# SeanNobel/DALLE2-video

Hardware: AMD Instinct MI355X
Metric: Unet3D denoise-steps/sec, 16f×64×64 clip bs=4; 1/2/4/8 MI355X (higher is better)
Workload: dtype bf16; 1 GPU; BASELINE config 2: unet1 (dim 64, mults 1/2/4/8) train step on a 16x64x64 clip, bs=4 per GPU: p_losses fwd+bwd + RCCL grad all-reduce + fused AdamW; batch_per_gpu=4, global_batch=4, parallelism=dp1

## Files before the change

### dalle2-video_amd/csrc/dv_conv.hip

```cpp
#include "dv_common.h"

#include <type_traits>

#include <algorithm>
#include <cstdlib>

using namespace dv;

#ifdef DV_STAMP
constexpr int DV_NSTAMP = 8;
__device__ unsigned long long g_dv_stamp[16384 * DV_NSTAMP];
#define DV_STAMP_AT(i)                                                                  \
  do {                                                                                  \
    if (threadIdx.x == 0) {                                                             \
      const long long blin = blockIdx.x + (long long)gridDim.x * (blockIdx.y + (long long)gridDim.y * blockIdx.z); \
      if (blin < 16384) g_dv_stamp[blin * DV_NSTAMP + (i)] = __builtin_amdgcn_s_memrealtime(); \
    }                                                                                   \
  } while (0)
extern "C" int dv_debug_stamps(unsigned long long* host, long long n) {
  if (n > 16384 * DV_NSTAMP) n = 16384 * DV_NSTAMP;
  return hipMemcpyFromSymbol(host, HIP_SYMBOL(g_dv_stamp), n * 8, 0, hipMemcpyDeviceToHost) == hipSuccess ? 0 : -1;
}
#else
#define DV_STAMP_AT(i) \
// ... 1908 lines not shown
    });
    if constexpr (GNIN) if (tr) {
      int ot = tid;
      asm volatile("" : "+v"(ot));
      const int gx = ot >> 3, gc = ot & 7;
#pragma unroll
      for (int i = 0; i < SEG; ++i) {
        const int q = (st + 1) * SEG + 2 + i, y = yq0 + q;
        const bool in = (unsigned)y < (unsigned)p.H;
        const u32x4 ov = in ? tv[i] : u32x4{0u, 0u, 0u, 0u};
        asm volatile("ds_write_b128 %0, %1" ::"v"(lds_addr(smem + (q % R) * ROWB + (gx + 1) * FS_XP + gc * 16)),
                     "v"(ov) : "memory");
        const bool own = in && q <= nst * SEG;
        __builtin_amdgcn_raw_buffer_store_b128(
            ov, yr, own ? (unsigned)(((fbase + y * W + gx) * p.gi_ldy + gc * 8) * 2) : DMA_OOB, 0, 0);
      }
    }
#ifdef DV_STAMP
    if (st == 1) {
      asm volatile("s_nop 0" : "+v"(acc));
      DV_S1(4);
    }
#endif
    const bool silu = p.act == DV_ACT_SILU;
    float sv[stats ? 32 : 1];
    const unsigned gba = lds_addr(gi_bias + ch * 32 + 4 * h);
#pragma unroll
    for (int g = 0; g < 4; ++g) {
      const int n = ch * 32 + 8 * g + 4 * h;
      float v[4];
#pragma unroll
      for (int e = 0; e < 4; ++e) v[e] = acc[4 * g + e];
      if constexpr (GNIN) {
        u32x4 gb = ds_read_b128_off<0>(gba + 32 * g);
        lgkm_wait_tied<0>(gb);
        const f32x4 bb = __builtin_bit_cast(f32x4, gb);
#pragma unroll
        for (int e = 0; e < 4; ++e) v[e] += bb[e];
      }
      if (silu) {
#pragma unroll
        for (int e = 0; e < 4; ++e) v[e] = silu_f(v[e]);
      }
      if (NRES > 0) {
#pragma unroll
        for (int e = 0; e < 4; ++e) v[e] += (float)rv[g][e];
      }
      if (NRES > 1) {
#pragma unroll
        for (int e = 0; e < 4; ++e) v[e] += (float)rv2[g][e];
      }
      store4<bf16>(p.y + m * p.ldy + co0 + n, v);
      if constexpr (stats) {
#pragma unroll
        for (int e = 0; e < 4; ++e) {
          const float q = stored<bf16>(v[e]);
          sv[4 * g + e] = q;
          sv[16 + 4 * g + e] = q * q;
        }
      }
    }
    if constexpr (stats) {
      rs_step<32, 16>(sv, r);
#pragma unroll
      for (int i = 0; i < 16; ++i) sacc[i] += sv[i];
    }
    if (st == 1) DV_S1(5);
    if constexpr (GNIN) {
      if (st + 2 < nst) {
        constexpr int B0 = Y0 + SEG + 4, B1 = 2 * SEG + 8;
        static_assert(B0 + NPW <= 63 && B1 + NPW <= 63, "stripe vmcnt immediate out of range");
        const bool d3 = st + 3 < nst;
        if (st == 0) {
          if (d3) asm volatile("s_waitcnt vmcnt(%0)" ::"n"(B0 + NPW) : "memory");
          else asm volatile("s_waitcnt vmcnt(%0)" ::"n"(B0) : "memory");
        } else {
          if (d3) asm volatile("s_waitcnt vmcnt(%0)" ::"n"(B1 + NPW) : "memory");
          else asm volatile("s_waitcnt vmcnt(%0)" ::"n"(B1) : "memory");
        }
      }
      if (tr) asm volatile("s_waitcnt lgkmcnt(0)" ::: "memory");
    } else if (st + 1 < nst) {
      constexpr int NR = 4 * NRES;
      constexpr int A0 = NR + 4, A1 = 2 * NR + 8, A2 = 2 * NR + 12;
      static_assert(A1 + 2 * NPW <= 63 && A2 + 2 * NPW <= 63, "stripe vmcnt immediate out of range");
      const int nd = (st + 2 < nst) + (st + 3 < nst);
      if (st == 0) {
        if (nd == 2) asm volatile("s_waitcnt vmcnt(%0)" ::"n"(A0 + 2 * NPW) : "memory");
        else if (nd == 1) asm volatile("s_waitcnt vmcnt(%0)" ::"n"(A0 + NPW) : "memory");
        else asm volatile("s_waitcnt vmcnt(%0)" ::"n"(A0) : "memory");
      } else if (st == 1) {
        if (nd == 2) asm volatile("s_waitcnt vmcnt(%0)" ::"n"(A1 + 2 * NPW) : "memory");
        else if (nd == 1) asm volatile("s_waitcnt vmcnt(%0)" ::"n"(A1 + NPW) : "memory");
        else asm volatile("s_waitcnt vmcnt(%0)" ::"n"(A1) : "memory");
      } else {
        if (nd == 2) asm volatile("s_waitcnt vmcnt(%0)" ::"n"(A2 + 2 * NPW) : "memory");
        else if (nd == 1) asm volatile("s_waitcnt vmcnt(%0)" ::"n"(A2 + NPW) : "memory");
        else asm volatile("s_waitcnt vmcnt(%0)" ::"n"(A2) : "memory");
      }
    }
    if (st == 1) DV_S1(6);
    __builtin_amdgcn_s_barrier();
    if (st == 0) DV_STAMP_AT(2);
    if (st == 1) DV_S1(7);
  }
  DV_STAMP_AT(3);
  if constexpr (stats) {
    __shared__ float red[2 * 64];
    rs_tail();
    if (nst > 0) gn_block_add<bf16, 32>(p, sacc, (long long)(sbeg + nst - 1) * 128 / p.gn_P, chan, red, co0, 64);
  }
}

bool fwd_stripe_ok(long long M, int h, int w, int cin, bool split, int cout, int ks, int ld0) {
  return ks == 3 && cin == 64 && !split && cout % 64 == 0 && (w == 32 || w == 64 || w == 128) &&
         h % (128 / w) == 0 && M % 128 == 0 && ld0 % 8 == 0 && M * ld0 * 2 < (long long)DMA_OOB;
}

int launch_fwd_stripe(const ConvFwdArgs<bf16>& a, hipStream_t st) {
  const int nstages = (int)(a.M / 128);
  const int ct = a.cout / 64;
  int bx = 256 / ct;
  if (bx < 1) bx = 1;
  if (bx > nstages) bx = nstages;
  const int spf = a.H / (128 / a.W);
  int sps = (nstages + bx - 1) / bx;
  if (sps >= spf) sps = spf;
  else while (spf % sps) ++sps;
  bx = (nstages + sps - 1) / sps;
  dim3 grid(bx, ct);
  const int nres = a.res2 ? 2 : a.res ? 1 : 0;
  const bool stats = a.gn_sums != nullptr;
  if (a.gi_sums) {
    if (stats) conv_fwd_stripe_kernel<64, 0, true, true><<<grid, 512, 0, st>>>(a, nstages, sps);
    else conv_fwd_stripe_kernel<64, 0, false, true><<<grid, 512, 0, st>>>(a, nstages, sps);
    return check_launch("conv_fwd_stripe_gn_in");
  }
#define DV_FS(WW, RR) (stats ? conv_fwd_stripe_kernel<WW, RR, true><<<grid, 512, 0, st>>>(a, nstages, sps) \
                             : conv_fwd_stripe_kernel<WW, RR, false><<<grid, 512, 0, st>>>(a, nstages, sps))
#define DV_FSR(WW) (nres == 2 ? (void)conv_fwd_stripe_kernel<WW, 2, false><<<grid, 512, 0, st>>>(a, nstages, sps) \
                    : nres == 1 ? (void)conv_fwd_stripe_kernel<WW, 1, false><<<grid, 512, 0, st>>>(a, nstages, sps) \
                                : DV_FS(WW, 0))
  if (a.W == 64 && nres == 1 && stats) conv_fwd_stripe_kernel<64, 1, true><<<grid, 512, 0, st>>>(a, nstages, sps);
  else if (a.W == 64) DV_FSR(64);
  else if (a.W == 128) DV_FSR(128);
  else DV_FSR(32);
#undef DV_FSR
#undef DV_FS
  return check_launch("conv_fwd_stripe");
}


bool stripe_geom(int h, int w, int& seg, int& nseg);

constexpr int F2_WP = 592;
constexpr int F2_XP = 80;

template <int W, bool STATS = false>
__global__ __launch_bounds__(512) void conv_fwd_stripe2_kernel(ConvFwdArgs<bf16> p, int seg, int nseg) {
  constexpr int WP = W + 2;
  constexpr int NWIN = W == 8 ? 200 : (128 / W + 2) * WP;
  constexpr int WB = 64 * F2_WP, XB = NWIN * F2_XP;
  constexpr int BUF = WB + XB;
  constexpr int NLW = (64 * 36 + 511) / 512;
  constexpr int NLX = (NWIN * 4 + 511) / 512;
  __shared__ __attribute__((aligned(16))) char smem[2 * BUF];

  const int tid = threadIdx.x, lane = tid & 63;
  const int wave = __builtin_amdgcn_readfirstlane(tid >> 6);
  const int pt = wave & 3, ch = wave >> 2;
  const int co0 = blockIdx.y * 64;
  const long long m0 = (long long)blockIdx.x * 128;
  const int HW = p.H * W, segrows = (seg + 2) * WP;
  const int y0 = nseg > 1 ? 0 : (int)((m0 % HW) / W);

  int w_src[NLW], w_dst[NLW];
#pragma unroll
  for (int i = 0; i < NLW; ++i) {
    const int idx = tid + 512 * i;
    const int row = idx / 36, c = idx - row * 36;
    const bool ok = row < 64;
    w_src[i] = ok ? (co0 + row) * p.K + (c >> 2) * p.cin + (c & 3) * 8 : -1;
    w_dst[i] = row * F2_WP + c * 16;
  }
  int x_off[NLX], x_ry[NLX], x_dst[NLX], x_c[NLX];
#pragma unroll
  for (int i = 0; i < NLX; ++i) {
    const int idx = tid + 512 * i;
    const int px = idx >> 2, c = idx & 3;
    const int sg = px / segrows, rem = px - sg * segrows;
    const int ry = rem / WP, rx = rem - ry * WP;
    const bool ok = px < NWIN && sg < nseg && rx >= 1 && rx <= W;
    x_ry[i] = ok ? ry - 1 : -(1 << 20);
    x_off[i] = sg * seg * W + (ry - 1) * W + (rx - 1);
    x_dst[i] = px < NWIN ? px * F2_XP + c * 16 : -1;
    x_c[i] = c * 8;
  }
  u32x4 rw[NLW], rx_[NLX];
  auto load = [&](int hc) {
    const int ci = hc * 32;
    const bool first = ci < p.c0;
    const bf16* xb = first ? p.x0 + ci : p.x1 + (ci - p.c0);
    const int ld = first ? p.ld0 : p.ld1;
#pragma unroll
    for (int i = 0; i < NLW; ++i)
      if (w_src[i] >= 0) rw[i] = *(const u32x4*)(p.w + w_src[i] + ci);
#pragma unroll
    for (int i = 0; i < NLX; ++i) {
      const bool in = (unsigned)(y0 + x_ry[i]) < (unsigned)p.H;
      rx_[i] = in ? *(const u32x4*)(xb + (m0 + x_off[i]) * ld + x_c[i]) : u32x4{0u, 0u, 0u, 0u};
    }
  };
  auto store = [&](int buf) {
    char* b = smem + buf * BUF;
#pragma unroll
    for (int i = 0; i < NLW; ++i)
      if (w_src[i] >= 0) *(u32x4*)(b + w_dst[i]) = rw[i];
#pragma unroll
    for (int i = 0; i < NLX; ++i)
      if (x_dst[i] >= 0) *(u32x4*)(b + WB + x_dst[i]) = rx_[i];
  };

  const int r = lane & 31, h = lane >> 5;
  const int px = pt * 32 + r;
  const int sl = px / (seg * W), rl = px - sl * seg * W;
  const int wrow = sl * segrows + (rl / W) * WP + rl % W;
  const int aofs = (ch * 32 + r) * F2_WP + h * 16;
  const int bofs = WB + wrow * F2_XP + h * 16;

  f32x16 acc[1][1];
#pragma unroll
  for (int e = 0; e < 16; ++e) acc[0][0][e] = 0.f;
  const int nhc = p.cin / 32;
  load(0);
  store(0);
  __syncthreads();
  for (int hc = 0; hc < nhc; ++hc) {
    if (hc + 1 < nhc) load(hc + 1);
    const char* b = smem + (hc & 1) * BUF;
#pragma unroll
    for (int d = 0; d < 9; ++d) {
      const int toff = ((d / 3) * WP + (d % 3)) * F2_XP;
#pragma unroll
      for (int ks = 0; ks < 2; ++ks) {
        const u32x4 av = *(const u32x4*)(b + aofs + (d * 32 + ks * 16) * 2);
        const u32x4 bv = *(const u32x4*)(b + bofs + toff + ks * 32);
        acc[0][0] = Mma<bf16>::run(av, bv, acc[0][0]);
      }
    }
    if (hc + 1 < nhc) store((hc + 1) & 1);
    __syncthreads();
  }
  conv_epilogue<bf16, 1, 1, STATS>(p, acc, m0 + pt * 32, co0 + ch * 32, r, h, m0, 128, co0, 64,
                                   (float*)smem);
}

bool fwd_stripe2_ok(long long M, int h, int w, int cin, int c0, bool split, int cout, int ks, int& seg,
                    int& nseg) {
  if (ks != 3 || cin % 32 || (split && c0 % 32) || cout % 64 || M % 128 || !stripe_geom(h, w, seg, nseg))
    return false;
  return w == 8 || (w == 16 && (long long)cin * cout <= 256 * 256);
}

int launch_fwd_stripe2(const ConvFwdArgs<bf16>& a, int seg, int nseg, hipStream_t st) {
  dim3 grid((unsigned)(a.M / 128), a.cout / 64);
  switch (a.W) {
#define DV_S2(WW) (a.gn_sums ? conv_fwd_stripe2_kernel<WW, true><<<grid, 512, 0, st>>>(a, seg, nseg) \
                          : conv_fwd_stripe2_kernel<WW, false><<<grid, 512, 0, st>>>(a, seg, nseg))
    case 64: DV_S2(64); break;
    case 32: DV_S2(32); break;
    case 16: DV_S2(16); break;
    default: DV_S2(8); break;
#undef DV_S2
  }
  return check_launch("conv_fwd_stripe2");
}

constexpr int F8_WROW = 19;
template <int W, int CO = 64, int NWV = 4, int NB = 0>
struct FwGeom {
  static constexpr int CG = CO * (NWV / 4);
  static constexpr int NF = W == 8 ? 2 : 1;
  static constexpr int NWR = W == 8 ? 10 : 128 / W + 2;
  static constexpr int WQ = W == 8 ? 12 : W + 2;
  static constexpr int FPIX = NWR * WQ;
  static constexpr int WPIX = NF * FPIX;
  static constexpr int XPIECES = (WPIX * 3 + 63) / 64;
  static constexpr int WPC = (CG * F8_WROW + 63) / 64;
  static constexpr int PIECES = WPC + XPIECES;
  static constexpr int NPW = (PIECES + NWV - 1) / NWV;
  static constexpr int BUF = PIECES * 1024;
  static constexpr int NBUF = NB ? NB : ((160 * 1024 - 1024) / BUF >= 5 ? 5 : (160 * 1024 - 1024) / BUF);
};

template <int W>
__device__ __forceinline__ int fw_pix(int r) {
  const bool ga = r < 4 || (r >= 12 && r < 16) || (r >= 20 && r < 28);
  const int a = ga ? (r < 4 ? r : (r < 16 ? r - 8 : r - 12))
                   : (r < 12 ? r - 4 : (r < 20 ? r - 8 : r - 16));
  if constexpr (W == 8) return (2 * (a >> 3) + (ga ? 0 : 1)) * 8 + (a & 7);
  else if constexpr (W == 16) return (ga ? 0 : 16) + a;
  else return (ga ? 0 : 16) + a;
}

template <int W, bool STATS = false, int PF = 2, int DEFER = 0, int CO = 64, bool SPLIT = true, int NWV = 4,
          bool TS = false>
__global__ __launch_bounds__(NWV * 64) void conv_fwd_frame_kernel(ConvFwdArgs<bf16> p) {
  using G = FwGeom<W, CO, TS ? 4 : NWV>;
  constexpr int PIECES = G::PIECES, BUF = G::BUF, NBUF = G::NBUF, WQ = G::WQ;
  constexpr int NPW = (PIECES + NWV - 1) / NWV;
  constexpr int WPC = G::WPC, NJ = TS ? 1 : CO / 32, CG = G::CG;
  static_assert(NWV == 4 || (NWV == 8 && (TS || !STATS)), "the 8-wave 2*CO tile has no statistics epilogue");
  static_assert(!TS || (NWV == 8 && CO == 64), "the tap split runs 8 waves on a 64-channel tile");
  static_assert(NPW <= 9, "one DMA piece per tap");
  __shared__ __attribute__((aligned(1024))) char smem[NBUF * BUF];
  DV_STAMP_AT(0);
  const int tid = threadIdx.x, lane = tid & 63;
  const int wave = __builtin_amdgcn_readfirstlane(tid >> 6) & (NWV - 1);
  const int wq = wave & 3;
  const int chh = TS ? 0 : wave >> 2;
  const int half = TS ? wave >> 2 : 0;
  const int npx = (int)(p.M / 128), nblk = npx * (p.cout / CG);
  int L = blockIdx.x;
  int co0;
  long long m0;
  if (p.xcd_c > 0) {
    const int xc = p.xcd_c, xp = 8 / xc, x = L % 8, j = L / 8;
    const int tpc = (p.cout / CG) / xc, ppg = npx / xp;
    co0 = ((x / xp) * tpc + j / ppg) * CG;
    m0 = (long long)((x % xp) * ppg + j % ppg) * 128;
  } else {
    if (nblk % 8 == 0) L = (L % 8) * (nblk / 8) + L / 8;
    co0 = (L / npx) * CG;
    m0 = (long long)(L % npx) * 128;
  }
  const int cbeg = 0, cend = p.cin / 16;
  const int nch = cend - cbeg;
  const int HW = p.H * W;
  const int y0 = W == 8 ? 0 : (int)((m0 % HW) / W);
  const long long fb = W == 8 ? m0 : m0 - (m0 % HW) + (long long)y0 * W;

  unsigned voff0[NPW], voff1[NPW];
#pragma unroll
  for (int i = 0; i < NPW; ++i) {
    const int k = min(wave + NWV * i, PIECES - 1);
    voff0[i] = voff1[i] = DMA_OOB;
    if (k < WPC) {
      const int slot = k * 64 + lane, row = slot / F8_WROW, c = slot - row * F8_WROW;
      if (c < 18 && row < CG) voff0[i] = (unsigned)((((long long)co0 + row) * p.K + c * 8) * 2);
    } else {
      const int slot = (k - WPC) * 64 + lane, px = slot / 3, s = slot - px * 3;
      const int f = px / G::FPIX, rem = px - f * G::FPIX, wy = rem / WQ, wx = rem - wy * WQ;
      const int y = y0 + wy - 1;
      if (px < G::WPIX && s < 2 && wx >= 1 && wx <= W && y >= 0 && y < p.H &&
          (W == 8 || wy <= 128 / W + 1)) {
        const long long pix = fb + (long long)f * 64 + (long long)(wy - 1) * W + (wx - 1);
        voff0[i] = (unsigned)(pix * p.ld0 * 2 + s * 16);
        voff1[i] = (unsigned)(pix * p.ld1 * 2 + s * 16);
      }
    }
  }
  const __amdgpu_buffer_rsrc_t wr = dma_rsrc(p.w, (unsigned)((long long)p.cout * p.K * 2));
  const __amdgpu_buffer_rsrc_t xr0 = dma_rsrc(p.x0, (unsigned)(p.M * p.ld0 * 2));
  const __amdgpu_buffer_rsrc_t xr1 = dma_rsrc(p.x1, (unsigned)(p.M * p.ld1 * 2));
  auto issue1 = [&](int c, int i) {
    const int ci0 = c * 16;
    const bool first = ci0 < p.c0;
    char* b = smem + (c % NBUF) * BUF;
    const int k = min(wave + NWV * i, PIECES - 1);
    if (k < WPC) dma16s(wr, b + k * 1024, voff0[i], (unsigned)ci0 * 18);
    else if (!SPLIT || first) dma16s(xr0, b + k * 1024, voff0[i], (unsigned)ci0 * 2);
    else dma16s(xr1, b + k * 1024, voff1[i], (unsigned)(ci0 - p.c0) * 2);
  };
  auto issue = [&](int c) {
#pragma unroll
    for (int i = 0; i < NPW; ++i) issue1(c, i);
  };
  constexpr int AHEAD = NBUF - 1;
#pragma unroll
  for (int c = 0; c < AHEAD; ++c)
    if (c < nch) issue(cbeg + c);
  {
    const int pro = min(AHEAD, nch) - 1;
    if (pro >= 3) asm volatile("s_waitcnt vmcnt(%0)" ::"n"(3 * NPW) : "memory");
    else if (pro == 2) asm volatile("s_waitcnt vmcnt(%0)" ::"n"(2 * NPW) : "memory");
    else if (pro == 1) asm volatile("s_waitcnt vmcnt(%0)" ::"n"(NPW) : "memory");
    else asm volatile("s_waitcnt vmcnt(0)" ::: "memory");
  }
  __builtin_amdgcn_s_barrier();
  DV_STAMP_AT(1);
#ifdef DV_STAMP
  unsigned long long st_wait = 0, st_bar = 0;
  const unsigned long long st_l0 = __builtin_amdgcn_s_memtime();
#endif

  const int r = lane & 31, h = lane >> 5;
  const int pix = fw_pix<W>(r);
  const int tpx = wq * 32 + pix;
  const int wb = W == 8 ? (tpx >> 6) * G::FPIX + ((tpx & 63) >> 3) * WQ + (tpx & 7)
                        : (tpx / W) * WQ + tpx % W;
  const int bofs = WPC * 1024 + (wb * 3 + h) * 16;
  const int aofs = (chh * CO + r) * (F8_WROW * 16) + h * 16;
  f32x16 acc0, acc1, acc2, acc3;
#pragma unroll
  for (int e = 0; e < 16; ++e) acc0[e] = acc1[e] = acc2[e] = acc3[e] = 0.f;
  static_assert(DEFER <= 2, "at most the last two taps are deferred");
  u32x4 lb[2], la0[2], la1[2];
  auto run_deferred = [&](auto HALF) {
    constexpr int D1 = TS && decltype(HALF)::value == 0 ? 5 : 9;
#pragma unroll
    for (int t = 0; t < DEFER; ++t) {
      const int tap = D1 - DEFER + t;
      if (tap & 1) {
        acc2 = Mma<bf16>::run(la0[t], lb[t], acc2);
        if (CO == 64) acc3 = Mma<bf16>::run(la1[t], lb[t], acc3);
      } else {
        acc0 = Mma<bf16>::run(la0[t], lb[t], acc0);
        if (CO == 64) acc1 = Mma<bf16>::run(la1[t], lb[t], acc1);
      }
    }
  };
  auto defer_wait = [&]() {
    if (DEFER == 2 && CO == 64)
      asm volatile("s_waitcnt lgkmcnt(0)" : "+v"(lb[0]), "+v"(la0[0]), "+v"(la1[0]), "+v"(lb[1]), "+v"(la0[1]),
                   "+v"(la1[1])::"memory");
    else if (DEFER == 2)
      asm volatile("s_waitcnt lgkmcnt(0)" : "+v"(lb[0]), "+v"(la0[0]), "+v"(lb[1]), "+v"(la0[1])::"memory");
    else if (DEFER && CO == 64)
      asm volatile("s_waitcnt lgkmcnt(0)" : "+v"(lb[0]), "+v"(la0[0]), "+v"(la1[0])::"memory");
    else if (DEFER)
      asm volatile("s_waitcnt lgkmcnt(0)" : "+v"(lb[0]), "+v"(la0[0])::"memory");
    else
      asm volatile("s_waitcnt lgkmcnt(0)" ::: "memory");
  };
  auto chunk = [&](int c, auto PRE, auto HALF) {
    const char* b = smem + (c % NBUF) * BUF;
    constexpr int D0 = TS && decltype(HALF)::value == 1 ? 5 : 0;
    constexpr int D1 = TS && decltype(HALF)::value == 0 ? 5 : 9;
    constexpr int NS = PF + 1;
    u32x4 bq[NS], aq0[NS], aq1[NS];
    auto rd = [&](int d, int s) {
      const int T = ((d / 3) * WQ + (d % 3)) * 48;
      bq[s] = *(const u32x4*)(b + bofs + T);
      aq0[s] = *(const u32x4*)(b + aofs + d * 32);
      if (CO == 64) aq1[s] = *(const u32x4*)(b + aofs + 32 * F8_WROW * 16 + d * 32);
    };
#pragma unroll
    for (int d = D0; d < D0 + PF; ++d) rd(d, d % NS);
    if (DEFER && c > cbeg) run_deferred(HALF);
#pragma unroll
    for (int d = D0; d < D1; ++d) {
      if (d + PF < D1) rd(d + PF, (d + PF) % NS);
      if (DEFER && d >= D1 - DEFER) {
        const int t = d - (D1 - DEFER);
        lb[t] = bq[d % NS];
        la0[t] = aq0[d % NS];
        if (CO == 64) la1[t] = aq1[d % NS];
      } else if (d & 1) {
        acc2 = Mma<bf16>::run(aq0[d % NS], bq[d % NS], acc2);
        if (CO == 64) acc3 = Mma<bf16>::run(aq1[d % NS], bq[d % NS], acc3);
      } else {
        acc0 = Mma<bf16>::run(aq0[d % NS], bq[d % NS], acc0);
        if (CO == 64) acc1 = Mma<bf16>::run(aq1[d % NS], bq[d % NS], acc1);
      }
      if constexpr (decltype(PRE)::value) {
        if (d - D0 < NPW) issue1(c + AHEAD, d - D0);
      }
      __builtin_amdgcn_sched_barrier(0);
    }
#ifdef DV_STAMP
    const unsigned long long tw0 = __builtin_amdgcn_s_memtime();
#endif
    if constexpr (decltype(PRE)::value) {
      asm volatile("s_waitcnt vmcnt(%0)" ::"n"((AHEAD - 1) * NPW) : "memory");
    } else {
      const int young = min(c + AHEAD, cend - 1) - (c + 1);
      if (young >= 3) asm volatile("s_waitcnt vmcnt(%0)" ::"n"(3 * NPW) : "memory");
      else if (young == 2) asm volatile("s_waitcnt vmcnt(%0)" ::"n"(2 * NPW) : "memory");
      else if (young == 1) asm volatile("s_waitcnt vmcnt(%0)" ::"n"(NPW) : "memory");
      else asm volatile("s_waitcnt vmcnt(0)" ::: "memory");
    }
    if (DEFER) defer_wait();
#ifdef DV_STAMP
    const unsigned long long tw1 = __builtin_amdgcn_s_memtime();
#endif
    __builtin_amdgcn_s_barrier();
#ifdef DV_STAMP
    const unsigned long long tw2 = __builtin_amdgcn_s_memtime();
    st_wait += tw1 - tw0;
    st_bar += tw2 - tw1;
#endif
  };
  using H0 = std::integral_constant<int, 0>;
  using H1 = std::integral_constant<int, 1>;
  int c = cbeg;
  if (half == 0) {
    for (; c + AHEAD < cend; ++c) chunk(c, std::true_type{}, H0{});
    for (; c < cend; ++c) chunk(c, std::false_type{}, H0{});
    if (DEFER && nch > 0) run_deferred(H0{});
  } else {
    for (; c + AHEAD < cend; ++c) chunk(c, std::true_type{}, H1{});
    for (; c < cend; ++c) chunk(c, std::false_type{}, H1{});
    if (DEFER && nch > 0) run_deferred(H1{});
  }
  DV_STAMP_AT(2);
#ifdef DV_STAMP
#ifndef FRAME_STAMP_WAVE
#define FRAME_STAMP_WAVE 0
#endif
  if (threadIdx.x == 64 * (FRAME_STAMP_WAVE < NWV ? FRAME_STAMP_WAVE : NWV - 1)) {
    const long long blin = blockIdx.x + (long long)gridDim.x * (blockIdx.y + (long long)gridDim.y * blockIdx.z);
    if (blin < 16384) {
      g_dv_stamp[blin * DV_NSTAMP + 5] = st_wait;
      g_dv_stamp[blin * DV_NSTAMP + 6] = st_bar;
      g_dv_stamp[blin * DV_NSTAMP + 7] = __builtin_amdgcn_s_memtime() - st_l0;
    }
  }
#endif
  f32x16 fin[NJ];
  if constexpr (TS) {
    f32x16 keep, give;
#pragma unroll
    for (int e = 0; e < 16; ++e) {
      const float s0 = acc0[e] + acc2[e], s1 = acc1[e] + acc3[e];
      keep[e] = half ? s1 : s0;
      give[e] = half ? s0 : s1;
    }
    f32x4* xb = (f32x4*)smem;
#pragma unroll
    for (int g = 0; g < 4; ++g)
      xb[((half * 4 + wq) * 4 + g) * 64 + lane] = f32x4{give[4 * g], give[4 * g + 1], give[4 * g + 2], give[4 * g + 3]};
    __syncthreads();
#pragma unroll
    for (int g = 0; g < 4; ++g) {
      const f32x4 o = xb[(((1 - half) * 4 + wq) * 4 + g) * 64 + lane];
#pragma unroll
      for (int e = 0; e < 4; ++e) keep[4 * g + e] += o[e];
    }
    fin[0] = keep;
  } else {
#pragma unroll
    for (int j = 0; j < NJ; ++j)
#pragma unroll
      for (int e = 0; e < 16; ++e) fin[j][e] = j ? acc1[e] + acc3[e] : acc0[e] + acc2[e];
  }
  const long long m = m0 + tpx;
  const int cw = co0 + chh * CO + half * 32;
  constexpr int NSV = 32 * NJ;
  float sv[STATS ? NSV : 1];
  f32x4 bb[NJ][4];
  u32x2 rq[NJ][4], rq2[NJ][4];
  if (p.bias) {
#pragma unroll
    for (int j = 0; j < NJ; ++j)
#pragma unroll
      for (int g = 0; g < 4; ++g) bb[j][g] = *(const f32x4*)(p.bias + cw + 32 * j + 8 * g + 4 * h);
  }
  if (p.res) {
#pragma unroll
    for (int j = 0; j < NJ; ++j)
#pragma unroll
      for (int g = 0; g < 4; ++g) rq[j][g] = *(const u32x2*)(p.res + m * p.ldres + cw + 32 * j + 8 * g + 4 * h);
  }
  if (p.res2) {
#pragma unroll
    for (int j = 0; j < NJ; ++j)
#pragma unroll
      for (int g = 0; g < 4; ++g) rq2[j][g] = *(const u32x2*)(p.res2 + m * p.ldres2 + cw + 32 * j + 8 * g + 4 * h);
  }
#pragma unroll
  for (int j = 0; j < NJ; ++j) {
#pragma unroll
    for (int g = 0; g < 4; ++g) {
      const int n = cw + 32 * j + 8 * g + 4 * h;
      float v[4];
#pragma unroll
      for (int e = 0; e < 4; ++e) v[e] = fin[j][4 * g + e];
      if (p.bias) {
#pragma unroll
        for (int e = 0; e < 4; ++e) v[e] += bb[j][g][e];
      }
      if (p.act == DV_ACT_SILU) {
#pragma unroll
        for (int e = 0; e < 4; ++e) v[e] = silu_f(v[e]);
      }
      if (p.res) {
        const bf16x4 t4 = __builtin_bit_cast(bf16x4, rq[j][g]);
#pragma unroll
        for (int e = 0; e < 4; ++e) v[e] += (float)t4[e];
      }
      if (p.res2) {
        const bf16x4 t4 = __builtin_bit_cast(bf16x4, rq2[j][g]);
#pragma unroll
        for (int e = 0; e < 4; ++e) v[e] += (float)t4[e];
      }
      store4<bf16>(p.y + m * p.ldy + n, v);
      if constexpr (STATS) {
#pragma unroll
        for (int e = 0; e < 4; ++e) {
          const float q = stored<bf16>(v[e]);
          sv[16 * j + 4 * g + e] = q;
          sv[NSV / 2 + 16 * j + 4 * g + e] = q * q;
        }
      }
    }
  }
  if constexpr (STATS) {
    gn_rs_reduce<NSV>(sv, r);
    gn_block_add<bf16, NSV>(p, sv, m0 / p.gn_P, [&](int k) {
      return cw + 32 * (k / 16) + 8 * ((k % 16) / 4) + 4 * h + (k % 4);
    }, (float*)smem, co0, CG);
  }
#ifdef DV_STAMP
  asm volatile("s_waitcnt vmcnt(0)" ::: "memory");
#endif
  DV_STAMP_AT(4);
}

bool fwd_frame_ok(const ConvFwdArgs<bf16>& a, int h, int w) {
  const long long maxb = (long long)DMA_OOB;
  const bool geom = (h == 8 && w == 8) || ((w == 16 || w == 32 || w == 64) && (h * w) % 128 == 0);
  return a.ks == 3 && geom && a.cin % 16 == 0 && a.c0 % 16 == 0 && a.cout % 64 == 0 &&
         a.M % 128 == 0 && a.ld0 % 8 == 0 && a.ld1 % 8 == 0 && (a.ldy & 3) == 0 &&
         (a.res == nullptr || (a.ldres & 3) == 0) && (a.res2 == nullptr || (a.ldres2 & 3) == 0) &&
         a.M * a.ld0 * 2 < maxb &&
         a.M * a.ld1 * 2 < maxb && (long long)a.cout * a.K * 2 < maxb &&
         ((uintptr_t)a.x0 & 15) == 0 && ((uintptr_t)a.x1 & 15) == 0 && ((uintptr_t)a.w & 15) == 0;
}

int frame_xcd_split(const ConvFwdArgs<bf16>& a, int co) {
  const int ntco = a.cout / co, npx = (int)(a.M / 128);
  auto ok = [&](int xc) { return ntco % xc == 0 && npx % (8 / xc) == 0; };
  const double wb = (double)a.cout * a.K, xb = (double)a.M * a.cin;
  int best = 0;
  double bc = 0;
  for (int xc = 1; xc <= 8; xc *= 2) {
    if (!ok(xc)) continue;
    const double c = (8 / xc) * wb + xc * xb;
    if (!best || c < bc) { best = xc; bc = c; }
  }
  return best;
}

int launch_fwd_frame(const ConvFwdArgs<bf16>& a0, hipStream_t st) {
  ConvFwdArgs<bf16> a = a0;
  const int tiles64 = (int)(a.M / 128) * (a.cout / 64);
  const int co = tiles64 <= 128 ? 32 : 64;
  const bool w8 = a.W == 16 && co == 64 && !a.gn_sums && a.cout % 128 == 0 && (a.M / 128) * (a.cout / 64) > 256;
  a.xcd_c = frame_xcd_split(a, w8 ? 128 : co);
  const int nblk = (int)(a.M / 128) * (a.cout / (w8 ? 128 : co));
  if (w8) {
    if (a.c0 < a.cin) conv_fwd_frame_kernel<16, false, 3, 1, 64, true, 8><<<nblk, 512, 0, st>>>(a);
    else conv_fwd_frame_kernel<16, false, 3, 1, 64, false, 8><<<nblk, 512, 0, st>>>(a);
    return check_launch("conv_fwd_frame");
  }
  if (a.W == 8 && co == 64) {
#define DV_FTS(SP) (a.gn_sums ? conv_fwd_frame_kernel<8, true, 3, 1, 64, SP, 8, true><<<nblk, 512, 0, st>>>(a) \
                              : conv_fwd_frame_kernel<8, false, 3, 1, 64, SP, 8, true><<<nblk, 512, 0, st>>>(a))
    if (a.c0 < a.cin) DV_FTS(true);
    else DV_FTS(false);
#undef DV_FTS
    return check_launch("conv_fwd_frame");
  }
  switch (a.W) {
#define DV_FW5(WW, C, SP) (a.gn_sums ? conv_fwd_frame_kernel<WW, true, 3, 1, C, SP><<<nblk, 256, 0, st>>>(a) \
                                 : conv_fwd_frame_kernel<WW, false, 3, 1, C, SP><<<nblk, 256, 0, st>>>(a))
#define DV_FW4(WW, C) (a.c0 < a.cin ? DV_FW5(WW, C, true) : DV_FW5(WW, C, false))
#define DV_FW(WW) (co == 32 ? DV_FW4(WW, 32) : DV_FW4(WW, 64))
    case 8: DV_FW(8); break;
    case 16: DV_FW(16); break;
    case 32: DV_FW(32); break;
    default: DV_FW(64); break;
#undef DV_FW
#undef DV_FW4
#undef DV_FW5
  }
  return check_launch("conv_fwd_frame");
}

inline void glds_tile(long long M, int cout, int K, int& bm, int& bn) {
  bn = cout <= 64 ? 64 : 128;
  bm = bn == 64 ? 256 : 128;
  if (((M + bm - 1) / bm) * ((cout + bn - 1) / bn) < 512) bm = 128;
  if (bn == 128 && ((M + 127) / 128) * ((cout + 127) / 128) < 256) bm = 64;
  (void)K;
}

template <typename T>
void set_gn(ConvFwdArgs<T>& a, float* gn_sums, long long gn_P, int gn_R) {
  a.gn_sums = gn_sums;
  a.gn_P = gn_sums ? gn_P : 1;
  a.gn_R = gn_R > 0 ? gn_R : 1;
  a.gn_rstride = gn_sums ? (a.M / a.gn_P) * a.cout * 2 : 0;
}

template <typename T>
int conv_fwd_t(const void* x0, int ld0, int c0, const void* x1, int ld1, const void* w,
               const float* bias, const void* res, int ldres, const void* res2, int ldres2, void* y,
               int ldy, int nf, int h, int wd, int cin, int cout, int ks, int act, float* gn_sums,
               long long gn_P, int gn_R, hipStream_t st) {
  if (!res && res2) {
    res = res2; ldres = ldres2; res2 = nullptr; ldres2 = 0;
  }
  ConvFwdArgs<T> a;
  a.x0 = (const T*)x0; a.x1 = (const T*)(x1 ? x1 : x0); a.ld0 = ld0; a.ld1 = x1 ? ld1 : ld0;
  a.c0 = x1 ? c0 : cin; a.w = (const T*)w; a.bias = bias; a.res = (const T*)res;
  a.ldres = ldres; a.res2 = (const T*)res2; a.ldres2 = ldres2;
  a.y = (T*)y; a.ldy = ldy; a.H = h; a.W = wd; a.cin = cin; a.cout = cout;
  a.ks = ks; a.act = act; a.M = (long long)nf * h * wd; a.K = ks * ks * cin;
  set_gn(a, gn_sums, gn_P, gn_R);
  if (a.M == 0 || cout == 0) return DV_OK;
  if constexpr (sizeof(T) == 2) {
    if (x1 && c0 == 64 && cin == 128 && act == DV_ACT_NONE && (!gn_sums || (wd == 64 && gn_P % 128 == 0)) &&
        !res2 && ld1 % 8 == 0 &&
        fwd_stripe_ok(a.M, h, wd, 64, false, cout, ks, ld0) && a.M * ld1 * 2 < (long long)DMA_OOB &&
        (ldy & 3) == 0 && (res == nullptr || (ldres & 3) == 0)) {
      ConvFwdArgs<T> p1 = a;
      p1.cin = 64; p1.c0 = 64; p1.x1 = p1.x0; p1.ld1 = p1.ld0; p1.K = ks * ks * 64;
      p1.wcin = 128; p1.wc0 = 0;
      set_gn(p1, nullptr, 0, 0);
      const int rc = launch_fwd_stripe(p1, st);
      if (rc != DV_OK) return rc;
      ConvFwdArgs<T> p2 = p1;
      p2.x0 = a.x1; p2.ld0 = a.ld1; p2.x1 = a.x1; p2.ld1 = a.ld1; p2.wc0 = 64;
      p2.bias = nullptr; p2.res = a.y; p2.ldres = ldy;
      set_gn(p2, gn_sums, gn_P, gn_R);
      return launch_fwd_stripe(p2, st);
    }
    if (fwd_stripe_ok(a.M, h, wd, cin, x1 != nullptr, cout, ks, ld0) && (ldy & 3) == 0 &&
        (res == nullptr || ((ldres & 3) == 0 && !gn_sums)) && (res2 == nullptr || (ldres2 & 3) == 0) &&
        (!gn_sums || gn_P % 128 == 0))
      return launch_fwd_stripe(a, st);
    int seg, nseg;
    if (fwd_stripe2_ok(a.M, h, wd, cin, a.c0, x1 != nullptr, cout, ks, seg, nseg) &&
        a.M * std::max(ld0, x1 ? ld1 : 0) < (1ll << 31))
      return launch_fwd_stripe2(a, seg, nseg, st);
    if (conv1x1_ok(a, x1 != nullptr) && !res2) {
      if (cout == 64) return cin == 64 ? launch_conv1x1<64, 1>(a, st) : launch_conv1x1<64, 2>(a, st);
      return cin == 64 ? launch_conv1x1<128, 1>(a, st) : launch_conv1x1<128, 2>(a, st);
    }
    const long long maxld = ld0 > (x1 ? ld1 : 0) ? ld0 : ld1;
    if (cin % 64 == 0 && a.c0 % 64 == 0 && a.M * maxld < (1ll << 31) && (ks == 1 || ks == 3)) {
      int bm, bn;
      glds_tile(a.M, cout, a.K, bm, bn);
      if (bm == 256) return launch_fwd_glds<256, 64>(a, st);
      if (bn == 64) return launch_fwd_glds<128, 64>(a, st);
      if (bm == 64) return launch_fwd_glds<64, 128>(a, st);
      return launch_fwd_glds<128, 128>(a, st);
    }
  }
  const long long mt128 = (a.M + 127) / 128;
  int bn = cout <= 64 ? 64 : 128;
  int bm = 128;
  if (mt128 * ((cout + bn - 1) / bn) < 512) bm = 64;
  if (bm == 64 && bn == 128 && ((a.M + 63) / 64) * ((cout + 127) / 128) < 512) bn = 64;
  if (bm == 128 && bn == 128) return launch_fwd<T, 128, 128>(a, st);
  if (bm == 128 && bn == 64) return launch_fwd<T, 128, 64>(a, st);
  if (bm == 64 && bn == 128) return launch_fwd<T, 64, 128>(a, st);
  return launch_fwd<T, 64, 64>(a, st);
}

template <typename T, int BMC, int BNK>
int launch_wgrad(WgradArgs<T> a, hipStream_t st) {
  const int mt = (a.cout + BMC - 1) / BMC, nt = (a.K + BNK - 1) / BNK;
  long long want = 1024 / ((long long)mt * nt);
  if (want < 1) want = 1;
  long long per = (a.M + want - 1) / want;
  per = ((per + 255) / 256) * 256;
  if (per < 256) per = 256;
  unsigned splits;
  if (a.batch_pix > 0) {
    const long long nbatch = a.M / a.batch_pix;
    long long spb = (a.batch_pix + per - 1) / per;
    per = (a.batch_pix + spb - 1) / spb;
    a.splits_per_batch = (int)spb;
    splits = (unsigned)(nbatch * spb);
  } else {
    splits = (unsigned)((a.M + per - 1) / per);
  }
  a.pix_per_split = (int)per;
  dim3 grid(mt, nt, splits);
  conv_wgrad_kernel<T, BMC, BNK><<<grid, 256, 0, st>>>(a);
  return check_launch("conv_wgrad");
}

template <typename T>
int conv_wgrad_t(const void* dy, int lddy, const void* x0, int ld0, int c0, const void* x1,
                 int ld1, float* ws, float* db, int nf, int h, int w, int cin, int cout, int ks,
                 hipStream_t st, long long batch_pix = 0) {
  WgradArgs<T> a;
  a.db = db;
  a.dy = (const T*)dy; a.lddy = lddy; a.x0 = (const T*)x0; a.x1 = (const T*)(x1 ? x1 : x0);
  a.ld0 = ld0; a.ld1 = x1 ? ld1 : ld0; a.c0 = x1 ? c0 : cin; a.ws = ws; a.H = h; a.W = w;
  a.cin = cin; a.cout = cout; a.ks = ks; a.K = ks * ks * cin; a.M = (long long)nf * h * w;
  a.pix_per_split = 0;
  a.batch_pix = batch_pix;
  a.ws_bstride = (long long)cout * a.K;
  a.splits_per_batch = 1;
  if (a.M == 0) return DV_OK;
  if constexpr (sizeof(T) == 2) {
    const long long maxld = std::max<long long>(std::max(lddy, ld0), x1 ? ld1 : 0);
    if (a.M * maxld < (1ll << 31) && (long long)cout * a.K < (1ll << 31))
      return conv_wgrad_glds(dy, lddy, x0, ld0, c0, x1, ld1, ws, db, nf, h, w, cin, cout, ks, st,
                             batch_pix);
  }
  const bool small_co = cout <= 64;
  const bool small_k = a.K <= 64;
  if (small_co && small_k) return launch_wgrad<T, 64, 64>(a, st);
  if (small_co) return launch_wgrad<T, 64, 128>(a, st);
  if (small_k) return launch_wgrad<T, 128, 64>(a, st);
  return launch_wgrad<T, 128, 128>(a, st);
}

struct WgradSArgs {
  const bf16* dy;
  int lddy;
  const bf16* x0;
  const bf16* x1;
  int ld0, ld1, c0;
  float* part;
  float* dbpart;
  float* dw;
  float* db;
  int acc_w, acc_b, part_bf16;
  int H, cin, cout, K;
  int nstages, stages_per_split;
};

template <int NT>
__device__ __forceinline__ void wgrad_tile_store(const WgradSArgs& a, f32x16 (&acc)[NT], float accb, char* smem,
                                                 int half, int wq, int wm, int wn, int lane, int co0, int ci0,
                                                 bool do_bias, int bz) {

  float* red = (float*)smem;
  constexpr int PERW = (NT * 16 + 1) * 64;
  if (half == 1) {
#pragma unroll
    for (int d = 0; d < NT; ++d)
#pragma unroll
      for (int e4 = 0; e4 < 4; ++e4)
        *(f32x4*)(red + wq * PERW + (d * 4 + e4) * 256 + lane * 4) =
            f32x4{acc[d][4 * e4], acc[d][4 * e4 + 1], acc[d][4 * e4 + 2], acc[d][4 * e4 + 3]};
    red[wq * PERW + NT * 16 * 64 + lane] = accb;
  }
  __syncthreads();
  if (half == 0) {
#pragma unroll
    for (int d = 0; d < NT; ++d)
#pragma unroll
      for (int e4 = 0; e4 < 4; ++e4) {
        const f32x4 v = *(const f32x4*)(red + wq * PERW + (d * 4 + e4) * 256 + lane * 4);
#pragma unroll
        for (int k = 0; k < 4; ++k) acc[d][4 * e4 + k] += v[k];
        __builtin_amdgcn_sched_barrier(0);
      }
    accb += red[wq * PERW + NT * 16 * 64 + lane];
  }
  __syncthreads();
  DV_STAMP_AT(3);
  if (gridDim.z > 1 && a.part_bf16) {
    constexpr int TP = 32 * NT;
    bf16* tiles = (bf16*)smem;
    const int r = lane & 31, h = lane >> 5;
    if (half == 0) {
      bf16* tb = tiles + wq * 32 * TP;
#pragma unroll
      for (int d = 0; d < NT; ++d)
#pragma unroll
        for (int e = 0; e < 16; ++e) tb[((e & 3) + 8 * (e >> 2) + 4 * h) * TP + r * NT + d] = (bf16)acc[d][e];
    }
    __syncthreads();
    bf16* dstb = (bf16*)a.part + (long long)bz * a.cout * a.K;
    constexpr int CPR = TP / 8;
    for (int idx = threadIdx.x; idx < 4 * 32 * CPR; idx += 512) {
      const int t4 = idx / (32 * CPR), rem = idx - t4 * (32 * CPR);
      const int col = rem / CPR, j = rem - col * CPR;
      const u32x4 v = *(const u32x4*)(tiles + (t4 * 32 + col) * TP + 8 * j);
      const long long oi = (long long)(co0 + (t4 >> 1) * 32 + col) * a.K + (ci0 + (t4 & 1) * 32) * NT + 8 * j;
      *(u32x4*)(dstb + oi) = v;
    }
#ifdef DV_STAMP
    asm volatile("s_waitcnt vmcnt(0)" ::: "memory");
#endif
    DV_STAMP_AT(4);
    if (do_bias && half == 0 && lane < 32) a.dbpart[(long long)bz * a.cout + co0 + wm * 32 + lane] = accb;
    return;
  }

  const bool direct = gridDim.z == 1;
  const bool pbf = !direct && a.part_bf16;
  float* dst = direct ? a.dw : a.part + (pbf ? 0 : (long long)bz * a.cout * a.K);
  bf16* dstb = (bf16*)a.part + (long long)bz * a.cout * a.K;
  const int acc_o = direct && a.acc_w;
  const int r = lane & 31, h = lane >> 5;
  constexpr int TP = 32 * NT;
#pragma unroll
  for (int rnd = 0; rnd < 2; ++rnd) {
    float* tile = red + wn * (32 * TP);
    if (half == 0 && wm == rnd) {
#pragma unroll
      for (int d = 0; d < NT; ++d)
#pragma unroll
        for (int e = 0; e < 16; ++e) {
          const int col = (e & 3) + 8 * (e >> 2) + 4 * h;
          tile[col * TP + r * NT + d] = acc[d][e];
        }
    }
    __syncthreads();
    for (int idx = threadIdx.x; idx < 2 * 32 * (TP / 4); idx += 512) {
      const int t2 = idx / (32 * (TP / 4)), rem = idx - t2 * (32 * (TP / 4));
      const int col = rem / (TP / 4), j = rem - col * (TP / 4);
      f32x4 v = *(const f32x4*)(red + t2 * (32 * TP) + col * TP + 4 * j);
      const long long rowbase = (long long)(co0 + rnd * 32) * a.K + (ci0 + t2 * 32) * NT;
      const long long oi = rowbase + (long long)col * a.K + 4 * j;
      if (pbf) {
        const float t4[4] = {v[0], v[1], v[2], v[3]};
        store4<bf16>(dstb + oi, t4);
        continue;
      }
      f32x4* o = (f32x4*)(dst + oi);
      if (acc_o) v += *o;
      *o = v;
    }
    __syncthreads();
  }
#ifdef DV_STAMP
  asm volatile("s_waitcnt vmcnt(0)" ::: "memory");
#endif
  DV_STAMP_AT(4);
  if (do_bias && half == 0 && lane < 32) {
    const int co = co0 + wm * 32 + lane;
    if (direct) a.db[co] = a.acc_b ? a.db[co] + accb : accb;
    else a.dbpart[(long long)bz * a.cout + co] = accb;
  }
}

template <int NBUF = 2>
__global__ __launch_bounds__(512, 4) void conv_wgrad_1x1_kernel(WgradSArgs a) {
  constexpr int AIMG = 2 * 128 * 64, BHALF = 128 * 64, STG = AIMG + 2 * BHALF;
  constexpr int DPS = 4;
  constexpr int RED1 = 4 * (16 + 1) * 64 * 4;
  constexpr int RING = NBUF * STG;
  __shared__ __attribute__((aligned(1024))) char smem[RING > RED1 ? RING : RED1];

  DV_STAMP_AT(0);
  const int tid = threadIdx.x, lane = tid & 63;
  const int wave = __builtin_amdgcn_readfirstlane(tid >> 6);
  const int half = wave >> 2, wq = wave & 3, wm = wq >> 1, wn = wq & 1;
  const int co0 = blockIdx.x * 64, ci0 = blockIdx.y * 64;
  const int sbeg = blockIdx.z * a.stages_per_split;
  const int send = min(sbeg + a.stages_per_split, a.nstages);
  const int nst = send - sbeg;

  const int l4 = lane >> 2, c4 = lane & 3, drow = 16 * wave;
  const bool first = ci0 < a.c0;
  const int xld = first ? a.ld0 : a.ld1;
// ... 766 lines not shown
```

Before: 107.0 denoise-steps/s.

## Give each wave a 64-pixel tile with tap split in 8-wave W16 conv

Adds a T64 mode to the frame conv forward kernel. Each wave now computes a 64-pixel × 64-channel tile over half of the taps, so every A-fragment read feeds two B fragments (four MFMAs per tap instead of two). The two tap halves are then summed across wave pairs through shared memory before the epilogue. The aim is more MFMA work per LDS read in the 8-wave 128-channel W=16 path. In exchange it adds a cross-wave reduction with a __syncthreads, raises register pressure from the extra B fragments, and issues multiple DMA pieces per tap.

```diff
diff --git a/dalle2-video_amd/csrc/dv_conv.hip b/dalle2-video_amd/csrc/dv_conv.hip
--- a/dalle2-video_amd/csrc/dv_conv.hip
+++ b/dalle2-video_amd/csrc/dv_conv.hip
@@ -2234,24 +2234,33 @@
   else if constexpr (W == 16) return (ga ? 0 : 16) + a;
   else return (ga ? 0 : 16) + a;
 }
+template <int W>
+__device__ __forceinline__ int fw_win_ofs(int tpx, int h) {
+  using G = FwGeom<W>;
+  const int wb = W == 8 ? (tpx >> 6) * G::FPIX + ((tpx & 63) >> 3) * G::WQ + (tpx & 7)
+                        : (tpx / W) * G::WQ + tpx % W;
+  return (wb * 3 + h) * 16;
+}
 
 template <int W, bool STATS = false, int PF = 2, int DEFER = 0, int CO = 64, bool SPLIT = true, int NWV = 4,
-          bool TS = false>
+          bool TS = false, bool T64 = false>
 __global__ __launch_bounds__(NWV * 64) void conv_fwd_frame_kernel(ConvFwdArgs<bf16> p) {
   using G = FwGeom<W, CO, TS ? 4 : NWV>;
   constexpr int PIECES = G::PIECES, BUF = G::BUF, NBUF = G::NBUF, WQ = G::WQ;
   constexpr int NPW = (PIECES + NWV - 1) / NWV;
   constexpr int WPC = G::WPC, NJ = TS ? 1 : CO / 32, CG = G::CG;
-  static_assert(NWV == 4 || (NWV == 8 && (TS || !STATS)), "the 8-wave 2*CO tile has no statistics epilogue");
-  static_assert(!TS || (NWV == 8 && CO == 64), "the tap split runs 8 waves on a 64-channel tile");
-  static_assert(NPW <= 9, "one DMA piece per tap");
+  constexpr bool TSP = TS || T64;
+  static_assert(NWV == 4 ? !TSP : NWV == 8 && TS != T64, "8 waves: the tap split (TS) or the 64-pixel wave tile (T64)");
+  static_assert(!TSP || CO == 64, "TS and T64 run on 64-channel tiles");
+  static_assert(!T64 || (!STATS && DEFER <= 1), "the 2*CO-channel tile has no statistics epilogue");
+  static_assert(NPW <= (TSP ? 8 : 9), "one DMA piece per tap (two per tap of a tap half)");
   __shared__ __attribute__((aligned(1024))) char smem[NBUF * BUF];
   DV_STAMP_AT(0);
   const int tid = threadIdx.x, lane = tid & 63;
   const int wave = __builtin_amdgcn_readfirstlane(tid >> 6) & (NWV - 1);
-  const int wq = wave & 3;
-  const int chh = TS ? 0 : wave >> 2;
-  const int half = TS ? wave >> 2 : 0;
+  const int wq = T64 ? (wave & 1) * 2 : wave & 3;
+  const int chh = T64 ? wave >> 2 : 0;
+  const int half = TS ? wave >> 2 : T64 ? ((wave >> 1) ^ (wave >> 2)) & 1 : 0;
   const int npx = (int)(p.M / 128), nblk = npx * (p.cout / CG);
   int L = blockIdx.x;
   int co0;
@@ -2329,21 +2338,28 @@
   const int r = lane & 31, h = lane >> 5;
   const int pix = fw_pix<W>(r);
   const int tpx = wq * 32 + pix;
-  const int wb = W == 8 ? (tpx >> 6) * G::FPIX + ((tpx & 63) >> 3) * WQ + (tpx & 7)
-                        : (tpx / W) * WQ + tpx % W;
-  const int bofs = WPC * 1024 + (wb * 3 + h) * 16;
+  const int bofs = WPC * 1024 + fw_win_ofs<W>(tpx, h);
+  const int bofs1 = WPC * 1024 + fw_win_ofs<W>(tpx + 32, h);
   const int aofs = (chh * CO + r) * (F8_WROW * 16) + h * 16;
   f32x16 acc0, acc1, acc2, acc3;
 #pragma unroll
   for (int e = 0; e < 16; ++e) acc0[e] = acc1[e] = acc2[e] = acc3[e] = 0.f;
   static_assert(DEFER <= 2, "at most the last two taps are deferred");
-  u32x4 lb[2], la0[2], la1[2];
+  u32x4 lb[2], la0[2], la1[2], lc[1];
+  auto mma4 = [&](const u32x4& a0, const u32x4& a1, const u32x4& b0, const u32x4& b1) {
+    acc0 = Mma<bf16>::run(a0, b0, acc0);
+    acc1 = Mma<bf16>::run(a1, b0, acc1);
+    acc2 = Mma<bf16>::run(a0, b1, acc2);
+    acc3 = Mma<bf16>::run(a1, b1, acc3);
+  };
   auto run_deferred = [&](auto HALF) {
-    constexpr int D1 = TS && decltype(HALF)::value == 0 ? 5 : 9;
+    constexpr int D1 = TSP && decltype(HALF)::value == 0 ? 5 : 9;
 #pragma unroll
     for (int t = 0; t < DEFER; ++t) {
       const int tap = D1 - DEFER + t;
-      if (tap & 1) {
+      if constexpr (T64) {
+        mma4(la0[t], la1[t], lb[t], lc[t]);
+      } else if (tap & 1) {
         acc2 = Mma<bf16>::run(la0[t], lb[t], acc2);
         if (CO == 64) acc3 = Mma<bf16>::run(la1[t], lb[t], acc3);
       } else {
@@ -2353,7 +2369,9 @@
     }
   };
   auto defer_wait = [&]() {
-    if (DEFER == 2 && CO == 64)
+    if (DEFER && T64)
+      asm volatile("s_waitcnt lgkmcnt(0)" : "+v"(lb[0]), "+v"(lc[0]), "+v"(la0[0]), "+v"(la1[0])::"memory");
+    else if (DEFER == 2 && CO == 64)
       asm volatile("s_waitcnt lgkmcnt(0)" : "+v"(lb[0]), "+v"(la0[0]), "+v"(la1[0]), "+v"(lb[1]), "+v"(la0[1]),
                    "+v"(la1[1])::"memory");
     else if (DEFER == 2)
@@ -2367,13 +2385,15 @@
   };
   auto chunk = [&](int c, auto PRE, auto HALF) {
     const char* b = smem + (c % NBUF) * BUF;
-    constexpr int D0 = TS && decltype(HALF)::value == 1 ? 5 : 0;
-    constexpr int D1 = TS && decltype(HALF)::value == 0 ? 5 : 9;
+    constexpr int D0 = TSP && decltype(HALF)::value == 1 ? 5 : 0;
+    constexpr int D1 = TSP && decltype(HALF)::value == 0 ? 5 : 9;
+    constexpr int IPT = (NPW + (D1 - D0) - 1) / (D1 - D0);
     constexpr int NS = PF + 1;
-    u32x4 bq[NS], aq0[NS], aq1[NS];
+    u32x4 bq[NS], cq[T64 ? NS : 1], aq0[NS], aq1[NS];
     auto rd = [&](int d, int s) {
       const int T = ((d / 3) * WQ + (d % 3)) * 48;
       bq[s] = *(const u32x4*)(b + bofs + T);
+      if constexpr (T64) cq[s] = *(const u32x4*)(b + bofs1 + T);
       aq0[s] = *(const u32x4*)(b + aofs + d * 32);
       if (CO == 64) aq1[s] = *(const u32x4*)(b + aofs + 32 * F8_WROW * 16 + d * 32);
     };
@@ -2386,8 +2406,11 @@
       if (DEFER && d >= D1 - DEFER) {
         const int t = d - (D1 - DEFER);
         lb[t] = bq[d % NS];
+        if constexpr (T64) lc[t] = cq[d % NS];
         la0[t] = aq0[d % NS];
         if (CO == 64) la1[t] = aq1[d % NS];
+      } else if constexpr (T64) {
+        mma4(aq0[d % NS], aq1[d % NS], bq[d % NS], cq[d % NS]);
       } else if (d & 1) {
         acc2 = Mma<bf16>::run(aq0[d % NS], bq[d % NS], acc2);
         if (CO == 64) acc3 = Mma<bf16>::run(aq1[d % NS], bq[d % NS], acc3);
@@ -2396,7 +2419,9 @@
         if (CO == 64) acc1 = Mma<bf16>::run(aq1[d % NS], bq[d % NS], acc1);
       }
       if constexpr (decltype(PRE)::value) {
-        if (d - D0 < NPW) issue1(c + AHEAD, d - D0);
+#pragma unroll
+        for (int q = 0; q < IPT; ++q)
+          if ((d - D0) * IPT + q < NPW) issue1(c + AHEAD, (d - D0) * IPT + q);
       }
       __builtin_amdgcn_sched_barrier(0);
     }
@@ -2449,8 +2474,29 @@
     }
   }
 #endif
-  f32x16 fin[NJ];
-  if constexpr (TS) {
+  constexpr int NF = T64 ? 2 : NJ;
+  f32x16 fin[NF];
+  if constexpr (T64) {
+    f32x4* xb = (f32x4*)smem;
+#pragma unroll
+    for (int j = 0; j < 2; ++j) {
+      const f32x16& give = half ? (j ? acc2 : acc0) : (j ? acc3 : acc1);
+#pragma unroll
+      for (int g = 0; g < 4; ++g)
+        xb[((wave * 2 + j) * 4 + g) * 64 + lane] = f32x4{give[4 * g], give[4 * g + 1], give[4 * g + 2], give[4 * g + 3]};
+    }
+    __syncthreads();
+#pragma unroll
+    for (int j = 0; j < 2; ++j) {
+      fin[j] = half ? (j ? acc3 : acc1) : (j ? acc2 : acc0);
+#pragma unroll
+      for (int g = 0; g < 4; ++g) {
+        const f32x4 o = xb[(((wave ^ 2) * 2 + j) * 4 + g) * 64 + lane];
+#pragma unroll
+        for (int e = 0; e < 4; ++e) fin[j][4 * g + e] += o[e];
+      }
+    }
+  } else if constexpr (TS) {
     f32x16 keep, give;
 #pragma unroll
     for (int e = 0; e < 16; ++e) {
@@ -2476,35 +2522,36 @@
 #pragma unroll
       for (int e = 0; e < 16; ++e) fin[j][e] = j ? acc1[e] + acc3[e] : acc0[e] + acc2[e];
   }
-  const long long m = m0 + tpx;
   const int cw = co0 + chh * CO + half * 32;
+  auto mj = [&](int j) { return m0 + tpx + (T64 ? 32 * j : 0); };
+  auto cj = [&](int j) { return cw + (T64 ? 0 : 32 * j); };
   constexpr int NSV = 32 * NJ;
   float sv[STATS ? NSV : 1];
-  f32x4 bb[NJ][4];
-  u32x2 rq[NJ][4], rq2[NJ][4];
+  f32x4 bb[NF][4];
+  u32x2 rq[NF][4], rq2[NF][4];
   if (p.bias) {
 #pragma unroll
-    for (int j = 0; j < NJ; ++j)
-#pragma unroll
-      for (int g = 0; g < 4; ++g) bb[j][g] = *(const f32x4*)(p.bias + cw + 32 * j + 8 * g + 4 * h);
+    for (int j = 0; j < NF; ++j)
+#pragma unroll
+      for (int g = 0; g < 4; ++g) bb[j][g] = *(const f32x4*)(p.bias + cj(j) + 8 * g + 4 * h);
   }
   if (p.res) {
 #pragma unroll
-    for (int j = 0; j < NJ; ++j)
-#pragma unroll
-      for (int g = 0; g < 4; ++g) rq[j][g] = *(const u32x2*)(p.res + m * p.ldres + cw + 32 * j + 8 * g + 4 * h);
+    for (int j = 0; j < NF; ++j)
+#pragma unroll
+      for (int g = 0; g < 4; ++g) rq[j][g] = *(const u32x2*)(p.res + mj(j) * p.ldres + cj(j) + 8 * g + 4 * h);
   }
   if (p.res2) {
 #pragma unroll
-    for (int j = 0; j < NJ; ++j)
-#pragma unroll
-      for (int g = 0; g < 4; ++g) rq2[j][g] = *(const u32x2*)(p.res2 + m * p.ldres2 + cw + 32 * j + 8 * g + 4 * h);
-  }
-#pragma unroll
-  for (int j = 0; j < NJ; ++j) {
+    for (int j = 0; j < NF; ++j)
+#pragma unroll
+      for (int g = 0; g < 4; ++g) rq2[j][g] = *(const u32x2*)(p.res2 + mj(j) * p.ldres2 + cj(j) + 8 * g + 4 * h);
+  }
+#pragma unroll
+  for (int j = 0; j < NF; ++j) {
 #pragma unroll
     for (int g = 0; g < 4; ++g) {
-      const int n = cw + 32 * j + 8 * g + 4 * h;
+      const int n = cj(j) + 8 * g + 4 * h;
       float v[4];
 #pragma unroll
       for (int e = 0; e < 4; ++e) v[e] = fin[j][4 * g + e];
@@ -2526,7 +2573,7 @@
 #pragma unroll
         for (int e = 0; e < 4; ++e) v[e] += (float)t4[e];
       }
-      store4<bf16>(p.y + m * p.ldy + n, v);
+      store4<bf16>(p.y + mj(j) * p.ldy + n, v);
       if constexpr (STATS) {
 #pragma unroll
         for (int e = 0; e < 4; ++e) {
@@ -2582,8 +2629,8 @@
   a.xcd_c = frame_xcd_split(a, w8 ? 128 : co);
   const int nblk = (int)(a.M / 128) * (a.cout / (w8 ? 128 : co));
   if (w8) {
-    if (a.c0 < a.cin) conv_fwd_frame_kernel<16, false, 3, 1, 64, true, 8><<<nblk, 512, 0, st>>>(a);
-    else conv_fwd_frame_kernel<16, false, 3, 1, 64, false, 8><<<nblk, 512, 0, st>>>(a);
+    if (a.c0 < a.cin) conv_fwd_frame_kernel<16, false, 3, 1, 64, true, 8, false, true><<<nblk, 512, 0, st>>>(a);
+    else conv_fwd_frame_kernel<16, false, 3, 1, 64, false, 8, false, true><<<nblk, 512, 0, st>>>(a);
     return check_launch("conv_fwd_frame");
   }
   if (a.W == 8 && co == 64) {
```

New measurement: 106.7 denoise-steps/s. About the same (-0.3%).
